# kakao/buffalo

Measured on NVIDIA H100. Metric: interactions/sec (nnz/s) ALS d=128, higher is better.
Workload: dtype f32

## Files before the change

### buffalo_b200/csrc/als_fast.cuh

```cuda
#pragma once
#include <algorithm>
#include <map>

#include "als_explicit.cuh"
#include "als_generic.cuh"
#include "als_tc.cuh"
#include "bfl_common.cuh"

namespace bfl {

constexpr int FAST_WARPS = 16;
constexpr int FAST_THREADS = FAST_WARPS * 32;
constexpr int FAST_NCLASS = 8;
constexpr int FAST_NR_CAP = 12288;

struct FastClass { int W, K, res, cap; };
__host__ __device__ inline FastClass fast_class(int c) {
    switch (c) {
        case 0: return {1, 1, 1, 32};
        case 1: return {1, 2, 1, 64};
        case 2: return {2, 2, 1, 128};
        case 3: return {4, 2, 1, 256};
        case 4: return {8, 2, 1, 512};
        case 5: return {16, 3, 1, 1536};
        case 6: return {16, 1, 0, FAST_NR_CAP};
        default: return {0, 0, 0, 0x7fffffff};
    }
}
__host__ __device__ inline int fast_class_of(int64_t n) {
    if (n <= 32) return 0;
    if (n <= 64) return 1;
    if (n <= 128) return 2;
    if (n <= 256) return 3;
    if (n <= 512) return 4;
    if (n <= 1536) return 5;
    if (n <= FAST_NR_CAP) return 6;
    return 7;
}

__host__ __device__ inline int fast_route(int64_t n, int long_regather) {
    const int c = fast_class_of(n);
    return (long_regather && c == 5) ? 6 : c;
}

__global__ void fast_count_kernel(const int64_t* __restrict__ indptr, int64_t row_begin, int64_t row_end,
                                  unsigned int* __restrict__ counts, int long_regather) {
    __shared__ unsigned int c[FAST_NCLASS];
    if (threadIdx.x < FAST_NCLASS) c[threadIdx.x] = 0;
    __syncthreads();
    for (int64_t r = row_begin + (int64_t)blockIdx.x * blockDim.x + threadIdx.x; r < row_end;
         r += (int64_t)gridDim.x * blockDim.x) {
        const int64_t n = indptr[r] - (r == 0 ? 0 : indptr[r - 1]);
        if (n > 0) atomicAdd(&c[fast_route(n, long_regather)], 1u);
    }
    __syncthreads();
    if (threadIdx.x < FAST_NCLASS && c[threadIdx.x]) atomicAdd(counts + threadIdx.x, c[threadIdx.x]);
}

__global__ void fast_fill_kernel(const int64_t* __restrict__ indptr, int64_t row_begin, int64_t row_end,
                                 unsigned int* __restrict__ cursors, int32_t* __restrict__ lists, int long_regather) {
    for (int64_t r = row_begin + (int64_t)blockIdx.x * blockDim.x + threadIdx.x; r < row_end;
         r += (int64_t)gridDim.x * blockDim.x) {
        const int64_t n = indptr[r] - (r == 0 ? 0 : indptr[r - 1]);
        if (n > 0) {
            const unsigned int pos = atomicAdd(cursors + fast_route(n, long_regather), 1u);
            lists[pos] = (int32_t)r;
        }
    }
}

template <int W>
__device__ __forceinline__ void team_sync(int team) {
    if (W == 1) {
        __syncwarp();
    } else {
        asm volatile("bar.sync %0, %1;" ::"r"(team + 1), "r"(32 * W) : "memory");
    }
}

__device__ __forceinline__ float4 ldg4(const float* p) { return __ldg(reinterpret_cast<const float4*>(p)); }
__device__ __forceinline__ float4 lds4(const float* p) { return *reinterpret_cast<const float4*>(p); }

__device__ __forceinline__ float2 ffma2(float2 a, float2 b, float2 c) {
    return make_float2(fmaf(a.x, b.x, c.x), fmaf(a.y, b.y, c.y));
}
__device__ __forceinline__ float2 fmul2(float2 a, float2 b) { return make_float2(__fmul_rn(a.x, b.x), __fmul_rn(a.y, b.y)); }

struct V8 { float2 v[4]; };

__device__ __forceinline__ V8 v8_zero() {
    V8 r;
#pragma unroll
    for (int k = 0; k < 4; ++k) r.v[k] = make_float2(0.f, 0.f);
    return r;
}
__device__ __forceinline__ V8 v8_from(float4 lo, float4 hi) {
    V8 r;
    r.v[0] = make_float2(lo.x, lo.y); r.v[1] = make_float2(lo.z, lo.w);
    r.v[2] = make_float2(hi.x, hi.y); r.v[3] = make_float2(hi.z, hi.w);
    return r;
}
__device__ __forceinline__ V8 v8_lds(const float* p) { return v8_from(lds4(p), lds4(p + 4)); }
__device__ __forceinline__ V8 v8_ldg(const float* p) { return v8_from(ldg4(p), ldg4(p + 4)); }
__device__ __forceinline__ float v8_dot(const V8& q, const V8& x) {
    float2 s = fmul2(q.v[0], x.v[0]);
#pragma unroll
    for (int k = 1; k < 4; ++k) s = ffma2(q.v[k], x.v[k], s);
    return s.x + s.y;
}
__device__ __forceinline__ void v8_axpy(V8& acc, float cf, const V8& q) {
    const float2 c2 = make_float2(cf, cf);
#pragma unroll
    for (int k = 0; k < 4; ++k) acc.v[k] = ffma2(c2, q.v[k], acc.v[k]);
}

__device__ __forceinline__ float transposed_reduce8(const V8& acc, int la) {
    const bool h4 = la & 4, h2 = la & 2, h1 = la & 1;
    const float2 s0 = h4 ? acc.v[0] : acc.v[2], s1 = h4 ? acc.v[1] : acc.v[3];
    const float2 k0 = h4 ? acc.v[2] : acc.v[0], k1 = h4 ? acc.v[3] : acc.v[1];
    float2 v0, v1;
    v0.x = k0.x + __shfl_xor_sync(FULL, s0.x, 16);
    v0.y = k0.y + __shfl_xor_sync(FULL, s0.y, 16);
    v1.x = k1.x + __shfl_xor_sync(FULL, s1.x, 16);
    v1.y = k1.y + __shfl_xor_sync(FULL, s1.y, 16);
    const float2 s = h2 ? v0 : v1, k = h2 ? v1 : v0;
    float2 u;
    u.x = k.x + __shfl_xor_sync(FULL, s.x, 8);
    u.y = k.y + __shfl_xor_sync(FULL, s.y, 8);
    return (h1 ? u.y : u.x) + __shfl_xor_sync(FULL, h1 ? u.x : u.y, 4);
}

__device__ __forceinline__ float sum_over_b(float s) {
    s += __shfl_xor_sync(FULL, s, 1);
    s += __shfl_xor_sync(FULL, s, 2);
    return s;
}

__device__ __forceinline__ void cp_async16(void* smem_dst, const void* gsrc) {
    asm volatile("cp.async.cg.shared.global [%0], [%1], 16;" ::"r"(smem_u32(smem_dst)), "l"(gsrc) : "memory");
}
__device__ __forceinline__ void cp_async_commit() { asm volatile("cp.async.commit_group;" ::: "memory"); }
__device__ __forceinline__ void cp_async_wait_all() { asm volatile("cp.async.wait_group 0;" ::: "memory"); }
__device__ __forceinline__ void prefetch_l2(const void* p) { asm volatile("prefetch.global.L2 [%0];" ::"l"(p)); }

__host__ __device__ inline size_t fast_team_floats(int D, int W, int cap) { return (size_t)D + 96 * W + 96 + 3 * (size_t)cap; }
__host__ __device__ inline size_t fast_smem_bytes(int D, int W, int K, int KS, bool res, bool gsm, int cap) {
    return sizeof(float) * ((gsm ? (size_t)D * (D + 4) : 0) + (res ? (size_t)FAST_WARPS * (K + KS) * 8 * 128 : 0) +
                            (FAST_WARPS / W) * fast_team_floats(D, W, cap));
}

template <int W, int K, int KS, bool RES, bool GSM, bool DET = false>
__global__ void __launch_bounds__(FAST_THREADS, 1) als_ialspp_team_kernel(AlsArgs a, int cap) {
    extern __shared__ __align__(16) float smem[];
    constexpr int TEAMS = FAST_WARPS / W;
    constexpr int KT = K + KS;
    const int D = a.D, ld = a.ld, GP = GSM ? D + 4 : D, NB = D >> 5;
    const int tid = threadIdx.x, lane = tid & 31;
    const int warp = __shfl_sync(FULL, tid >> 5, 0);
// ... 411 lines not shown
        const int g7 = (int)std::min<int64_t>((n7 + 127) / 128, 1024);
        if (BFL_OK != fb->chunk_end.reserve((size_t)n7)) return BFL_ERR_CUDA;
        tc::tc_chunk_counts_kernel<<<g7, 128, 0, st>>>(a0.indptr, list7, n7, TC_SPLIT, fb->chunk_end.p);
        BFL_LAUNCHED();
        int rc = inclusive_scan_i64(fb->chunk_end.p, fb->chunk_end.p, n7, st);
        if (rc != BFL_OK) return rc;
        fb->h_chunk_end.resize((size_t)n7);
        BFL_CUDA(cudaMemcpyAsync(fb->h_chunk_end.data(), fb->chunk_end.p, sizeof(long long) * (size_t)n7, cudaMemcpyDeviceToHost, st));
        BFL_CUDA(cudaStreamSynchronize(st));
        const long long total = fb->h_chunk_end.back();
        if (BFL_OK != fb->items.reserve(3 * (size_t)total)) return BFL_ERR_CUDA;
        tc::tc_fill_items_scanned_kernel<<<g7, 128, 0, st>>>(list7, n7, fb->chunk_end.p, fb->items.p);
        BFL_LAUNCHED();
        fb->n_items = (int64_t)total;
        fb->items_split_class = split_min_class;
        fb->items_det = true;
        fb->det_batches.clear();
    }
    const size_t sf = tc::scratch_floats<D>(), sfb = sf * sizeof(float);
    if (!cache.det_budget) {
        size_t free_b = 0, total_b = 0;
        BFL_CUDA(cudaMemGetInfo(&free_b, &total_b));
        cache.det_budget = std::max<size_t>(std::min<size_t>(free_b / 4, (size_t)2 << 30), 2 * sfb);
    }
    const long long* ce = fb->h_chunk_end.data();
    if (fb->det_batches.empty() || fb->det_batches_budget != cache.det_budget) {
        fb->det_batches.assign(1, 0);
        size_t used = 0;
        for (int64_t i = 0; i < n7; ++i) {
            const size_t cost = (size_t)(ce[i] - (i ? ce[i - 1] : 0) + 1) * sfb;
            if (used && used + cost > cache.det_budget) {
                fb->det_batches.push_back(i);
                used = 0;
            }
            used += cost;
        }
        fb->det_batches.push_back(n7);
        fb->det_batches_budget = cache.det_budget;
    }
    int64_t max_rows = 0, max_chunks = 0;
    for (size_t b = 0; b + 1 < fb->det_batches.size(); ++b) {
        const int64_t i = fb->det_batches[b], j = fb->det_batches[b + 1];
        max_rows = std::max(max_rows, j - i);
        max_chunks = std::max<int64_t>(max_chunks, ce[j - 1] - (i ? ce[i - 1] : 0));
    }
    if (BFL_OK != cache.scratch.reserve(sf * (size_t)max_rows) || BFL_OK != cache.chunk_scratch.reserve(sf * (size_t)max_chunks))
        BFL_FAIL(BFL_ERR_CUDA, "deterministic ALS: cannot allocate the split-row scratch (" +
                                   std::to_string((sfb * (size_t)(max_rows + max_chunks)) >> 20) +
                                   " MB); lower _b200_det_scratch_mb or free device memory");
    const int nf4 = (int)((a0.compute_loss && a0.axis == 1 ? sf : (size_t)D * D + D) / 4);
    for (size_t b = 0; b + 1 < fb->det_batches.size(); ++b) {
        const int64_t i = fb->det_batches[b], j = fb->det_batches[b + 1];
        const int64_t chunk0 = i ? ce[i - 1] : 0, nchunks = ce[j - 1] - chunk0;
        int rc = tc::tc_launch_partial<D>(a0, fb->items.p + 3 * chunk0, nchunks, cache.chunk_scratch.p, nchunks, TC_SPLIT,
                                          num_sms, st, true);
        if (rc != BFL_OK) return rc;
        for (int64_t r = i; r < j; r += 65535) {
            const dim3 grid((nf4 + 255) / 256, (unsigned)std::min<int64_t>(65535, j - r));
            tc::tc_chunk_reduce_kernel<<<grid, 256, 0, st>>>(cache.chunk_scratch.p, fb->chunk_end.p, r, chunk0, sf, nf4,
                                                             cache.scratch.p + (size_t)(r - i) * sf);
            BFL_LAUNCHED();
        }
        rc = launch_explicit_solve(a0, list7 + i, j - i, cache.scratch.p, det_loss, num_sms, st);
        if (rc != BFL_OK) return rc;
    }
    return BFL_OK;
}

inline int fast_als_launch(const AlsArgs& a0, FastCache& cache, int num_sms, cudaStream_t st,
                           const int32_t** leftover_rows, int64_t* leftover_count, int tc_min_class, int split_min_class,
                           int long_regather = 0, bool det = false) {
    const bool det_loss = det && a0.loss && a0.compute_loss;
    *leftover_rows = nullptr;
    *leftover_count = 0;
    const int64_t nrows = a0.row_end - a0.row_begin;
    FastBinKey key{a0.indptr, a0.row_begin, a0.row_end};
    FastBins* fb = nullptr;
    auto it = cache.bins.find(key);
    if (it == cache.bins.end()) {
        if (cache.bins.size() >= 256) cache.clear();
        fb = new FastBins();
        if (BFL_OK != fb->lists.reserve((size_t)nrows) || BFL_OK != fb->counters.reserve(2 * FAST_NCLASS)) {
            delete fb;
            return BFL_ERR_CUDA;
        }
        BFL_CUDA(cudaMemsetAsync(fb->counters.p, 0, 2 * FAST_NCLASS * sizeof(unsigned int), st));
        const int grid = (int)std::min<int64_t>((nrows + 255) / 256, (int64_t)num_sms * 8);
        fast_count_kernel<<<grid, 256, 0, st>>>(a0.indptr, a0.row_begin, a0.row_end, fb->counters.p, long_regather);
        BFL_LAUNCHED();
        BFL_CUDA(cudaMemcpyAsync(fb->count, fb->counters.p, FAST_NCLASS * sizeof(unsigned int), cudaMemcpyDeviceToHost, st));
        BFL_CUDA(cudaStreamSynchronize(st));
        fb->offset[0] = 0;
        for (int c = 0; c < FAST_NCLASS; ++c) fb->offset[c + 1] = fb->offset[c] + fb->count[c];
        BFL_CUDA(cudaMemcpyAsync(fb->counters.p + FAST_NCLASS, fb->offset, FAST_NCLASS * sizeof(unsigned int),
                                 cudaMemcpyHostToDevice, st));
        fast_fill_kernel<<<grid, 256, 0, st>>>(a0.indptr, a0.row_begin, a0.row_end, fb->counters.p + FAST_NCLASS,
                                               fb->lists.p, long_regather);
        BFL_LAUNCHED();
        cache.bins[key] = fb;
    } else {
        fb = it->second;
    }
    tc_min_class = std::min(tc_min_class, split_min_class);
    const bool has_split = split_min_class < FAST_NCLASS && fb->offset[FAST_NCLASS] > fb->offset[split_min_class];
    if (has_split && det) {
        const int64_t n7 = fb->offset[FAST_NCLASS] - fb->offset[split_min_class];
        const int32_t* list7 = fb->lists.p + fb->offset[split_min_class];
        const int rc = a0.D == 128
                           ? fast_split_rows_det<128>(a0, cache, fb, list7, n7, split_min_class, det_loss, num_sms, st)
                           : fast_split_rows_det<256>(a0, cache, fb, list7, n7, split_min_class, det_loss, num_sms, st);
        if (rc != BFL_OK) return rc;
    }
    if (has_split && !det) {
        const int64_t n7 = fb->offset[FAST_NCLASS] - fb->offset[split_min_class];
        const int32_t* list7 = fb->lists.p + fb->offset[split_min_class];
        if (fb->n_items < 0 || fb->items_split_class != split_min_class) {
            if (BFL_OK != fb->item_counter.reserve(2)) return BFL_ERR_CUDA;
            BFL_CUDA(cudaMemsetAsync(fb->item_counter.p, 0, 2 * sizeof(unsigned long long), st));
            const int g7 = (int)std::min<int64_t>((n7 + 127) / 128, 1024);
            tc::tc_count_items_kernel<<<g7, 128, 0, st>>>(a0.indptr, list7, n7, TC_SPLIT, fb->item_counter.p);
            BFL_LAUNCHED();
            unsigned long long total = 0;
            BFL_CUDA(cudaMemcpyAsync(&total, fb->item_counter.p, sizeof(total), cudaMemcpyDeviceToHost, st));
            BFL_CUDA(cudaStreamSynchronize(st));
            if (BFL_OK != fb->items.reserve(3 * (size_t)total)) return BFL_ERR_CUDA;
            tc::tc_fill_items_kernel<<<g7, 128, 0, st>>>(a0.indptr, list7, n7, TC_SPLIT, fb->item_counter.p + 1, fb->items.p);
            BFL_LAUNCHED();
            fb->n_items = (int64_t)total;
            fb->items_split_class = split_min_class;
        }
        const size_t sf = a0.D == 128 ? tc::scratch_floats<128>() : tc::scratch_floats<256>();
        if (BFL_OK != cache.scratch.reserve(sf * (size_t)n7)) return BFL_ERR_CUDA;
        int rc = a0.D == 128
                     ? tc::tc_launch_partial<128>(a0, fb->items.p, fb->n_items, cache.scratch.p, n7, TC_SPLIT, num_sms, st)
                     : tc::tc_launch_partial<256>(a0, fb->items.p, fb->n_items, cache.scratch.p, n7, TC_SPLIT, num_sms, st);
        if (rc != BFL_OK) return rc;
        rc = launch_explicit_solve(a0, list7, n7, cache.scratch.p, false, num_sms, st);
        if (rc != BFL_OK) return rc;
    }
    if (tc_min_class < split_min_class && fb->offset[split_min_class] > fb->offset[tc_min_class]) {
        AlsArgs a = a0;
        a.row_list = fb->lists.p;
        a.row_begin = fb->offset[tc_min_class];
        a.row_end = fb->offset[split_min_class];
        const int rc = tc::tc_launch(a, num_sms, st, det_loss);
        if (rc != BFL_OK) return rc;
    }
    for (int c = 0; c < std::min(FAST_NCLASS - 1, tc_min_class); ++c) {
        if (!fb->count[c]) continue;
        AlsArgs a = a0;
        a.row_list = fb->lists.p;
        a.row_begin = fb->offset[c];
        a.row_end = fb->offset[c + 1];
        const FastClass fc = fast_class(c);
        int rc = BFL_OK;
        const bool gsm = a.D <= 128;
        switch (c) {
            case 0: rc = gsm ? fast_launch_class<1, 1, 0, true, true>(a, fc.cap, num_sms, st, det_loss)
                             : fast_launch_class<1, 1, 0, true, false>(a, fc.cap, num_sms, st, det_loss); break;
            case 1: rc = gsm ? fast_launch_class<1, 2, 0, true, true>(a, fc.cap, num_sms, st, det_loss)
                             : fast_launch_class<1, 2, 0, true, false>(a, fc.cap, num_sms, st, det_loss); break;
            case 2: rc = gsm ? fast_launch_class<2, 2, 0, true, true>(a, fc.cap, num_sms, st, det_loss)
                             : fast_launch_class<2, 2, 0, true, false>(a, fc.cap, num_sms, st, det_loss); break;
            case 3: rc = gsm ? fast_launch_class<4, 2, 0, true, true>(a, fc.cap, num_sms, st, det_loss)
                             : fast_launch_class<4, 2, 0, true, false>(a, fc.cap, num_sms, st, det_loss); break;
            case 4: rc = gsm ? fast_launch_class<8, 2, 0, true, true>(a, fc.cap, num_sms, st, det_loss)
                             : fast_launch_class<8, 2, 0, true, false>(a, fc.cap, num_sms, st, det_loss); break;
            case 5: rc = fast_launch_class<16, 2, 1, true, false>(a, fc.cap, num_sms, st, det_loss); break;
            case 6: rc = gsm ? fast_launch_class<16, 1, 0, false, true>(a, fc.cap, num_sms, st, det_loss)
                             : fast_launch_class<16, 1, 0, false, false>(a, fc.cap, num_sms, st, det_loss); break;
        }
        if (rc != BFL_OK) return rc;
    }
    if (split_min_class >= FAST_NCLASS && fb->count[FAST_NCLASS - 1]) {
        *leftover_rows = fb->lists.p + fb->offset[FAST_NCLASS - 1];
        *leftover_count = fb->count[FAST_NCLASS - 1];
    }
    return BFL_OK;
}

}
```

### buffalo_b200/csrc/als_tc.cuh

```cuda
#pragma once
#include "als_generic.cuh"
#include "bfl_common.cuh"
#include <type_traits>

#include "sm90_ptx.cuh"

namespace bfl {
namespace tc {

using namespace sm90;

constexpr int N_CONV = 4, KH = N_CONV / 4;
constexpr int W_EPI = 0, W_MMA = 4, W_CONV = 8, W_PLAN = W_CONV + N_CONV;
constexpr int WARPS = 16, THREADS = WARPS * 32;
constexpr int REG_MMA = 200, REG_PLAN = 4 * 128 - 128 - 128 - REG_MMA;
constexpr int NXS = 8;
constexpr int PT = 2;
constexpr int NR = 2;
constexpr int NO = 2;
constexpr int GATHER_AHEAD = 1;
constexpr int NPG = 8, NP = NPG * PT;
constexpr int NBV = 8;
template <int D>
struct Cfg {
    static constexpr int TILE = D == 128 ? 32 : 16;
    static constexpr int NF = D / 128;
    static constexpr int LBO = D * 16;
    static constexpr int OP_BYTES = TILE * D * 2;
};
constexpr uint32_t F_FIRST = 1u << 8, F_LAST = 1u << 9, F_NEG = 1u << 10, F_STOP = 1u << 11;

__device__ __forceinline__ int msw(int c) { return ((c >> 1) & 3) << 3; }

template <int D>
struct Smem {
    static constexpr int TILE = Cfg<D>::TILE;
    alignas(1024) unsigned char op[NO][PT][2][Cfg<D>::OP_BYTES];
    alignas(128) float raw[NR][PT][TILE * D];
    alignas(128) float mat[128 * 128];
    alignas(16) float bvec[NBV][KH][D];
    alignas(16) float sumq[NBV][KH][D];
    alignas(16) float xs[NXS][D];
    alignas(16) float pv[4][32];
    alignas(16) float dl[4][32];
    alignas(16) float sws[NP][TILE];
    alignas(16) float wv[NP][TILE];
    alignas(16) int32_t keys[NP][TILE];
    float wsum[NBV][KH];
    uint32_t meta_raw[NP];
    uint32_t meta_op[NO][PT];
    int badrow[NXS];
    alignas(8) uint64_t plan_full[NPG], plan_empty[NPG], raw_full[NR], raw_empty[NR], op_full[NO], op_empty[NO];
    alignas(8) uint64_t acc_full, acc_empty, x_full[NXS], d_full[4];
};
template <int D>
struct SmemDet : Smem<D> {
    double lossp[NXS][4][2];
};

struct TcArgs {
    AlsArgs a;
    const int32_t* items;
    float* scratch;
    int64_t split;
    int pass;
    int debug;
};

template <int D>
__host__ __device__ constexpr size_t scratch_floats() { return (size_t)D * D + 2 * D + 4; }

__global__ void tc_absmax_kernel(const float* __restrict__ p, size_t n, unsigned int* __restrict__ out) {
    float m = 0.f;
    const size_t gtid = (size_t)blockIdx.x * blockDim.x + threadIdx.x, gsz = (size_t)gridDim.x * blockDim.x;
    const size_t lead = min(n, (size_t)(((16 - ((uintptr_t)p & 15)) & 15) / 4));
    const size_t n4 = (n - lead) / 4;
    const float4* p4 = reinterpret_cast<const float4*>(p + lead);
    for (size_t i = gtid; i < n4; i += gsz) {
        const float4 v = __ldg(p4 + i);
        m = fmaxf(fmaxf(m, fmaxf(fabsf(v.x), fabsf(v.y))), fmaxf(fabsf(v.z), fabsf(v.w)));
    }
    for (size_t i = gtid; i < lead; i += gsz) m = fmaxf(m, fabsf(p[i]));
    for (size_t i = lead + n4 * 4 + gtid; i < n; i += gsz) m = fmaxf(m, fabsf(p[i]));
    for (int o = 16; o > 0; o >>= 1) m = fmaxf(m, __shfl_xor_sync(FULL, m, o));
    if ((threadIdx.x & 31) == 0 && m > 0.f) atomicMax(out, __float_as_uint(m));
}
__global__ void tc_scale_kernel(const unsigned int* __restrict__ ymax, const unsigned int* __restrict__ vmax, float alpha,
                                float* __restrict__ out) {
    const float y = __uint_as_float(*ymax), w = __uint_as_float(*vmax) * fabsf(alpha);
    const float top = y * sqrtf(w);
    int e = 0;
    if (top > 0.f && isfinite(top)) {
        int ex;
        frexpf(top, &ex);
        e = 15 - ex;
    }
    e = max(-60, min(60, e));
    out[0] = ldexpf(1.f, e);
    out[1] = ldexpf(1.f, -2 * e);
}

template <int D, bool PARTIAL, bool LOSS1, bool DET = false>
__global__ void __launch_bounds__(THREADS, 1) als_tc_kernel(TcArgs ta) {
    static_assert(D == 128 || (D == 256 && PARTIAL), "fused row solve: d = 128; split-row mode: d = 128 or 256");
    constexpr int TILE = Cfg<D>::TILE, NF = Cfg<D>::NF, LBO = Cfg<D>::LBO;
    extern __shared__ __align__(1024) unsigned char smem_raw_[];
    Smem<D>& S = *reinterpret_cast<Smem<D>*>(smem_raw_);
    [[maybe_unused]] SmemDet<D>& SD = *reinterpret_cast<SmemDet<D>*>(smem_raw_);
    const AlsArgs& a = ta.a;
    const int tid = threadIdx.x, lane = tid & 31;
    const int warp = __shfl_sync(FULL, tid >> 5, 0);

    if (tid == 0) {
        for (int i = 0; i < NR; ++i) {
            mbar_init(&S.raw_full[i], N_CONV);
            mbar_init(&S.raw_empty[i], N_CONV);
        }
        for (int i = 0; i < NPG; ++i) {
            mbar_init(&S.plan_full[i], 1);
            mbar_init(&S.plan_empty[i], N_CONV);
        }
        for (int i = 0; i < NO; ++i) {
            mbar_init(&S.op_full[i], N_CONV);
            mbar_init(&S.op_empty[i], 4);
        }
        mbar_init(&S.acc_full, 4);
        mbar_init(&S.acc_empty, 4);
        for (int b = 0; b < 4; ++b) mbar_init(&S.d_full[b], 1);
        for (int i = 0; i < NXS; ++i) {
            mbar_init(&S.x_full[i], 4);
            S.badrow[i] = 0;
        }
        mbar_init_fence();
    }
    __syncthreads();
    const float scale = __ldg(a.tc_scales), inv2 = __ldg(a.tc_scales + 1);

    const int64_t nitems = a.row_end - a.row_begin;
    const int64_t my_first = (int64_t)blockIdx.x;
    const int64_t stride = gridDim.x;

    auto item_info = [&](int64_t it, int& row, int64_t& beg, int64_t& n, int& slot) {
        if (PARTIAL) {
            const int32_t* p = ta.items + 3 * (a.row_begin + it);
            row = p[0];
            const int64_t rb = row == 0 ? 0 : a.indptr[row - 1];
            const int64_t rn = a.indptr[row] - rb;
            beg = rb + (int64_t)p[1] * ta.split;
            n = min(ta.split, rn - (int64_t)p[1] * ta.split);
            slot = DET ? (int)it : p[2];
        } else {
            row = a.row_list[a.row_begin + it];
            beg = row == 0 ? 0 : a.indptr[row - 1];
            n = a.indptr[row] - beg;
            slot = 0;
        }
    };

    if (warp >= W_PLAN) {
        setmaxnreg_dec<REG_PLAN>();
        if (warp != W_PLAN) return;
        uint32_t gsl = 0, rph = 0, pe = 0;
        auto tile_begin = [&]() -> uint32_t {
            if (pe == 0) mbar_wait_idle(&S.plan_empty[gsl], rph ^ 1u);
            return gsl * PT + pe;
        };
        auto tile_end = [&]() {
            if (++pe == PT) {
                if (lane == 0) mbar_arrive(&S.plan_full[gsl]);
                pe = 0;
                if (++gsl == NPG) { gsl = 0; rph ^= 1u; }
            }
        };
        auto emit = [&](unsigned mask, uint32_t flags, int32_t key, float w) {
            const int cnt = __popc(mask);
            const int slot = __popc(mask & ((1u << lane) - 1u));
            const uint32_t rs = tile_begin();
            if ((mask >> lane) & 1u) {
                S.keys[rs][slot] = key;
                S.sws[rs][slot] = sqrtf(fabsf(w)) * scale;
                S.wv[rs][slot] = w;
            } else {
                const int zslot = cnt + lane - slot;
                if (zslot < TILE) {
                    S.sws[rs][zslot] = 0.f;
                    S.wv[rs][zslot] = 0.f;
                }
            }
            if (lane == 0) S.meta_raw[rs] = (uint32_t)cnt | flags;
            __syncwarp();
            tile_end();
        };
        constexpr int SC = 4, SCN = SC * TILE;
        const bool inl = lane < TILE;
        auto load_id = [&](int64_t it, int& row, int& chunk) {
            row = -1;
            chunk = 0;
            if (it < nitems) {
                if (PARTIAL) {
                    const int32_t* p = ta.items + 3 * (a.row_begin + it);
                    row = p[0];
                    chunk = p[1];
                } else {
                    row = a.row_list[a.row_begin + it];
                }
            }
        };
        auto load_span = [&](int row, int chunk, const int32_t*& kp, const float*& vp, int& n) {
            kp = a.keys;
            vp = a.vals;
            n = 0;
            if (row >= 0) {
                const int64_t rb = row == 0 ? 0 : a.indptr[row - 1];
                const int64_t rn = a.indptr[row] - rb;
                int64_t beg = rb;
                n = (int)rn;
                if (PARTIAL) {
                    beg = rb + (int64_t)chunk * ta.split;
                    n = (int)min(ta.split, rn - (int64_t)chunk * ta.split);
                }
                kp = a.keys + (beg - a.shift);
                vp = a.vals + (beg - a.shift);
            }
        };
        auto load_sc = [&](const int32_t* kp, const float* vp, int n, int c0, int32_t (&key)[SC], float (&w)[SC]) {
#pragma unroll
            for (int s = 0; s < SC; ++s) {
                const int idx = c0 + s * TILE + lane;
                const bool ok = inl && idx < n;
                key[s] = ok ? kp[idx] : 0;
                w[s] = ok ? vp[idx] * a.alpha : 0.f;
            }
        };
        auto emit_sc = [&](int n, int c0, const int32_t (&key)[SC], const float (&w)[SC]) {
            bool neg = false;
#pragma unroll
            for (int s = 0; s < SC; ++s) neg |= w[s] < 0.f;
            if (!__any_sync(FULL, neg)) {
#pragma unroll
                for (int s = 0; s < SC; ++s) {
                    const int t0 = c0 + s * TILE;
                    if (t0 < n) {
                        const uint32_t meta = (uint32_t)min(TILE, n - t0) | (t0 == 0 ? F_FIRST : 0u) | (t0 + TILE >= n ? F_LAST : 0u);
                        const uint32_t rs = tile_begin();
                        if (inl) {
                            float sq;
                            asm("sqrt.approx.ftz.f32 %0, %1;" : "=f"(sq) : "f"(w[s]));
                            S.keys[rs][lane] = key[s];
                            S.sws[rs][lane] = sq * scale;
                            S.wv[rs][lane] = w[s];
                        }
                        if (lane == 0) S.meta_raw[rs] = meta;
                        __syncwarp();
                        tile_end();
// ... 434 lines not shown
            if (++os == NO) { os = 0; oph ^= 1u; }
        }
    } else {
        const int q = warp & 3;
        const int j = q * 32 + lane;
        float* pv = S.pv[q];
        double l_nume = 0.0, l_deno = 0.0;
        const float tol = a.tol;
        if constexpr (PARTIAL) {
            int row = 0, slot = 0, nrow = 0, nslot = 0;
            int64_t beg, n = 0, nbeg, nn = 0;
            if (my_first < nitems) item_info(my_first, row, beg, n, slot);
            for (int64_t seq = 0; my_first + seq * stride < nitems; ++seq) {
                const int64_t nit = my_first + (seq + 1) * stride;
                if (nit < nitems) item_info(nit, nrow, nbeg, nn, nslot);
                const uint32_t aph = (uint32_t)(seq & 1);
                const uint32_t bs = (uint32_t)(seq & (NBV - 1));
                mbar_wait_idle(&S.acc_full, aph);
                float* sc = ta.scratch + (size_t)slot * scratch_floats<D>();
                if constexpr (DET) {
                    if (ta.pass == 0) {
                        for (int jj = j; jj < D; jj += 128) {
                            sc[(size_t)D * D + jj] = S.bvec[bs][0][jj] + (KH == 2 ? S.bvec[bs][KH - 1][jj] : 0.f);
                            if (LOSS1) sc[(size_t)D * D + D + jj] = S.sumq[bs][0][jj] + (KH == 2 ? S.sumq[bs][KH - 1][jj] : 0.f);
                        }
                        if (LOSS1 && j < 4)
                            sc[(size_t)D * D + 2 * D + j] = j == 0 ? S.wsum[bs][0] + (KH == 2 ? S.wsum[bs][KH - 1] : 0.f) : 0.f;
                    }
                } else if (ta.pass == 0) {
                    for (int jj = j; jj < D; jj += 128) {
                        atomicAdd(sc + (size_t)D * D + jj, S.bvec[bs][0][jj] + (KH == 2 ? S.bvec[bs][KH - 1][jj] : 0.f));
                        if (LOSS1) atomicAdd(sc + (size_t)D * D + D + jj, S.sumq[bs][0][jj] + (KH == 2 ? S.sumq[bs][KH - 1][jj] : 0.f));
                    }
                    if (LOSS1 && j == 0) atomicAdd(sc + (size_t)D * D + 2 * D, S.wsum[bs][0] + (KH == 2 ? S.wsum[bs][KH - 1] : 0.f));
                }
                __syncwarp();
                if (lane == 0) mbar_arrive(&S.acc_empty);
                row = nrow; slot = nslot; n = nn;
            }
        } else {
            auto row_of = [&](int64_t sq) -> int {
                const int64_t it = my_first + sq * stride;
                return it < nitems ? a.row_list[a.row_begin + it] : -1;
            };
            auto len_of = [&](int row) -> float {
                if (row < 0 || !a.compute_loss) return 0.f;
                return (float)(a.indptr[row] - (row == 0 ? 0 : a.indptr[row - 1]));
            };
            int row = (ta.debug & 16) ? -1 : row_of(0), row1 = row_of(1), row2 = row_of(2);
            float xj = row >= 0 ? a.X[(int64_t)row * a.ld + j] : 0.f;
            float x1 = row1 >= 0 ? a.X[(int64_t)row1 * a.ld + j] : 0.f;
            float nlen = len_of(row), nlen1 = len_of(row1);
            if (row >= 0) {
                S.xs[0][j] = xj;
                __syncwarp();
                if (lane == 0) mbar_arrive(&S.x_full[0]);
            }
            auto mat = [&](int c) -> float { return S.mat[c * 128 + (j ^ msw(c))]; };
            for (int64_t seq = 0; row >= 0; ++seq) {
                const int row3 = row_of(seq + 3);
                const float x2 = row2 >= 0 ? a.X[(int64_t)row2 * a.ld + j] : 0.f;
                const float nlen2 = len_of(row2);
                if (row1 >= 0) {
                    S.xs[(seq + 1) & (NXS - 1)][j] = x1;
                    __syncwarp();
                    if (lane == 0) mbar_arrive(&S.x_full[(seq + 1) & (NXS - 1)]);
                }
                const uint32_t aph = (uint32_t)(seq & 1);
                const uint32_t bs = (uint32_t)(seq & (NBV - 1));
                const uint32_t xsl = (uint32_t)(seq & (NXS - 1));
                const float* xs = S.xs[xsl];
                mbar_wait(&S.x_full[xsl], (uint32_t)((seq / NXS) & 1));
                mbar_wait_idle(&S.acc_full, aph);
                if (ta.debug & 8) {
                    __syncwarp();
                    if (lane == 0) mbar_arrive(&S.acc_empty);
                    row = row1; row1 = row2; row2 = row3;
                    xj = x1; x1 = x2;
                    continue;
                }
                const float bj = S.bvec[bs][0][j] + (KH == 2 ? S.bvec[bs][KH - 1][j] : 0.f);
                double ln_row = 0.0, ld_row = 0.0;
                float hM = 0.f;
                float md[32];
#pragma unroll
                for (int c = 0; c < D / 32; ++c) {
                    float h0 = 0.f, h1 = 0.f;
#pragma unroll
                    for (int i = 0; i < 32; i += 4) {
                        const float4 x4 = *reinterpret_cast<const float4*>(xs + c * 32 + i);
                        const float m0 = mat(c * 32 + i), m1 = mat(c * 32 + i + 1), m2 = mat(c * 32 + i + 2), m3 = mat(c * 32 + i + 3);
                        h0 = fmaf(m0, x4.x, h0); h1 = fmaf(m1, x4.y, h1);
                        h0 = fmaf(m2, x4.z, h0); h1 = fmaf(m3, x4.w, h1);
                        if (c == q) { md[i] = m0; md[i + 1] = m1; md[i + 2] = m2; md[i + 3] = m3; }
                    }
                    hM += h0 + h1;
                }
                if (a.compute_loss) {
                    const float kappa = a.adaptive_reg ? nlen : 1.0f;
                    double t = (double)(kappa * a.reg * xj * xj);
                    if (a.axis == 1) {
                        t += (double)xj * (double)hM - (double)(a.reg * xj * xj) -
                             2.0 * (double)xj * ((double)bj + (double)S.sumq[bs][0][j] + (KH == 2 ? (double)S.sumq[bs][KH - 1][j] : 0.0));
                        if (j == 0) {
                            const double ws = (double)S.wsum[bs][0] + (KH == 2 ? (double)S.wsum[bs][KH - 1] : 0.0);
                            t += (double)nlen + ws;
                            l_deno += (double)a.Y_rows + ws;
                        }
                    }
                    if constexpr (DET) {
                        ln_row = warp_sum_d(t);
                        ld_row = l_deno;
                        l_deno = 0.0;
                        if (q < 3 && lane == 0) {
                            SD.lossp[xsl][q][0] = ln_row;
                            SD.lossp[xsl][q][1] = ld_row;
                        }
                    } else {
                        l_nume += t;
                    }
                }
                float h = hM - bj;
#pragma unroll 1
                for (int B = 0; B < q; ++B) {
                    float mv[32];
#pragma unroll
                    for (int i = 0; i < 32; ++i) mv[i] = mat(B * 32 + i);
                    mbar_wait(&S.d_full[B], aph);
                    float u0 = 0.f, u1 = 0.f;
#pragma unroll
                    for (int i = 0; i < 32; i += 4) {
                        const float4 d4 = *reinterpret_cast<const float4*>(&S.dl[B][i]);
                        u0 = fmaf(mv[i], d4.x, u0);
                        u1 = fmaf(mv[i + 1], d4.y, u1);
                        u0 = fmaf(mv[i + 2], d4.z, u0);
                        u1 = fmaf(mv[i + 3], d4.w, u1);
                    }
                    h -= u0 + u1;
                }
                if constexpr (DET) {
                    if (q == 3 && lane == 0 && a.loss && a.compute_loss) {
                        double sn = SD.lossp[xsl][0][0], sd = SD.lossp[xsl][0][1];
#pragma unroll
                        for (int w = 1; w < 3; ++w) {
                            sn += SD.lossp[xsl][w][0];
                            sd += SD.lossp[xsl][w][1];
                        }
                        a.loss[2 * (int64_t)row] = sn + ln_row;
                        a.loss[2 * (int64_t)row + 1] = sd + ld_row;
                    }
                }
                __syncwarp();
                if (lane == 0) mbar_arrive(&S.acc_empty);
                float xv = 0.f;
                {
                    float r = h, p = h;
                    float rsold = warp_sum(r * r);
                    bool act = rsold > tol;
#pragma unroll 1
                    for (int step = 0; step < 3; ++step) {
                        pv[lane] = p;
                        __syncwarp();
                        float a0 = 0.f, a1 = 0.f, a2 = 0.f, a3 = 0.f;
#pragma unroll
                        for (int i = 0; i < 32; i += 4) {
                            const float4 p4 = *reinterpret_cast<const float4*>(pv + i);
                            a0 = fmaf(md[i], p4.x, a0); a1 = fmaf(md[i + 1], p4.y, a1);
                            a2 = fmaf(md[i + 2], p4.z, a2); a3 = fmaf(md[i + 3], p4.w, a3);
                        }
                        __syncwarp();
                        const float Ap = (a0 + a1) + (a2 + a3);
                        const float pAp = warp_sum(p * Ap);
                        const float ss = act ? __fdividef(rsold, pAp) : 0.f;
                        xv = fmaf(ss, p, xv);
                        r = fmaf(-ss, Ap, r);
                        const float rsnew = warp_sum(r * r);
                        act = act && !(rsnew < tol);
                        if (act) p = fmaf(__fdividef(rsnew, rsold), p, r);
                        rsold = act ? rsnew : rsold;
                    }
                }
                float v = xj - xv;
                const bool badw = __any_sync(FULL, !isfinite(v));
                a.X[(int64_t)row * a.ld + j] = v;
                for (int pr = 0; pr < a.n_peer; ++pr) a.peerX[pr][(int64_t)row * a.ld + j] = v;
                if (q < 3) {
                    S.dl[q][lane] = xv;
                    if (badw && lane == 0) atomicOr(&S.badrow[xsl], 1);
                    __syncwarp();
                    if (lane == 0) mbar_arrive(&S.d_full[q]);
                }
                if (q == 3) {
                    const bool bad = badw || (S.badrow[xsl] != 0);
                    if (bad) {
#pragma unroll
                        for (int c = 0; c < 4; ++c) {
                            a.X[(int64_t)row * a.ld + c * 32 + lane] = 0.f;
                            for (int pr = 0; pr < a.n_peer; ++pr) a.peerX[pr][(int64_t)row * a.ld + c * 32 + lane] = 0.f;
                        }
                        __syncwarp();
                        if (lane == 0) S.badrow[xsl] = 0;
                    }
                }
                row = row1; row1 = row2; row2 = row3;
                xj = x1; x1 = x2;
                nlen = nlen1; nlen1 = nlen2;
            }
            if (!DET && a.loss && a.compute_loss) {
                l_nume = warp_sum_d(l_nume);
                l_deno = warp_sum_d(l_deno);
                if (lane == 0 && (l_nume != 0.0 || l_deno != 0.0)) {
                    atomicAdd(a.loss, l_nume);
                    atomicAdd(a.loss + 1, l_deno);
                }
            }
        }
    }
}

inline bool tc_applicable(int optimizer_code, int d, int vdim, int block_size) {
    return optimizer_code == 8 && d == 128 && vdim == 128 && block_size == 32;
}
inline bool tc_split_applicable(int optimizer_code, int d, int vdim, int block_size) {
    return optimizer_code == 8 && (d == 128 || d == 256) && vdim == d && block_size == 32;
}

inline int tc_note_absmax(const float* p, size_t n, unsigned int* out, int num_sms, cudaStream_t st) {
    BFL_CUDA(cudaMemsetAsync(out, 0, sizeof(unsigned int), st));
    if (n == 0) return BFL_OK;
    const int grid = (int)std::min<size_t>((n / 4 + 255) / 256 + 1, (size_t)num_sms * 8);
    tc_absmax_kernel<<<grid, 256, 0, st>>>(p, n, out);
    BFL_LAUNCHED();
    return BFL_OK;
}
inline int tc_update_scale(const unsigned int* ymax, const unsigned int* vmax, float alpha, float* scales, cudaStream_t st) {
    tc_scale_kernel<<<1, 1, 0, st>>>(ymax, vmax, alpha, scales);
    BFL_LAUNCHED();
    return BFL_OK;
}

__global__ void tc_count_items_kernel(const int64_t* __restrict__ indptr, const int32_t* __restrict__ list, int64_t nrows,
                                      int64_t split, unsigned long long* total) {
    for (int64_t i = (int64_t)blockIdx.x * blockDim.x + threadIdx.x; i < nrows; i += (int64_t)gridDim.x * blockDim.x) {
        const int row = list[i];
        const int64_t n = indptr[row] - (row == 0 ? 0 : indptr[row - 1]);
        atomicAdd(total, (unsigned long long)((n + split - 1) / split));
    }
}
__global__ void tc_fill_items_kernel(const int64_t* __restrict__ indptr, const int32_t* __restrict__ list, int64_t nrows,
                                     int64_t split, unsigned long long* cursor, int32_t* __restrict__ items) {
    for (int64_t i = (int64_t)blockIdx.x * blockDim.x + threadIdx.x; i < nrows; i += (int64_t)gridDim.x * blockDim.x) {
        const int row = list[i];
        const int64_t n = indptr[row] - (row == 0 ? 0 : indptr[row - 1]);
        const int64_t nc = (n + split - 1) / split;
        const unsigned long long pos = atomicAdd(cursor, (unsigned long long)nc);
        for (int64_t c = 0; c < nc; ++c) {
            items[3 * (pos + c) + 0] = row;
            items[3 * (pos + c) + 1] = (int32_t)c;
            items[3 * (pos + c) + 2] = (int32_t)i;
        }
    }
}

__global__ void tc_chunk_counts_kernel(const int64_t* __restrict__ indptr, const int32_t* __restrict__ list, int64_t nrows,
                                       int64_t split, long long* __restrict__ counts) {
    for (int64_t i = (int64_t)blockIdx.x * blockDim.x + threadIdx.x; i < nrows; i += (int64_t)gridDim.x * blockDim.x) {
        const int row = list[i];
        const int64_t n = indptr[row] - (row == 0 ? 0 : indptr[row - 1]);
        counts[i] = (n + split - 1) / split;
    }
}
__global__ void tc_fill_items_scanned_kernel(const int32_t* __restrict__ list, int64_t nrows,
                                             const long long* __restrict__ chunk_end, int32_t* __restrict__ items) {
    for (int64_t i = (int64_t)blockIdx.x * blockDim.x + threadIdx.x; i < nrows; i += (int64_t)gridDim.x * blockDim.x) {
        const int64_t pos = i == 0 ? 0 : chunk_end[i - 1], nc = chunk_end[i] - pos;
        for (int64_t c = 0; c < nc; ++c) {
            items[3 * (pos + c) + 0] = list[i];
            items[3 * (pos + c) + 1] = (int32_t)c;
            items[3 * (pos + c) + 2] = (int32_t)i;
        }
    }
}

__global__ void __launch_bounds__(256) tc_chunk_reduce_kernel(const float* __restrict__ chunks, const long long* __restrict__ chunk_end,
                                                              int64_t row0, int64_t chunk0, size_t slot_floats, int nf4,
                                                              float* __restrict__ rows_out) {
    const int64_t i = row0 + blockIdx.y;
    const int64_t c0 = (i == 0 ? 0 : chunk_end[i - 1]) - chunk0, c1 = chunk_end[i] - chunk0;
    float4* out = reinterpret_cast<float4*>(rows_out + (size_t)blockIdx.y * slot_floats);
    for (int e = blockIdx.x * blockDim.x + threadIdx.x; e < nf4; e += gridDim.x * blockDim.x) {
        float4 acc = __ldg(reinterpret_cast<const float4*>(chunks + (size_t)c0 * slot_floats) + e);
        for (int64_t c = c0 + 1; c < c1; ++c) {
            const float4 v = __ldg(reinterpret_cast<const float4*>(chunks + (size_t)c * slot_floats) + e);
            acc.x = __fadd_rn(acc.x, v.x);
            acc.y = __fadd_rn(acc.y, v.y);
            acc.z = __fadd_rn(acc.z, v.z);
            acc.w = __fadd_rn(acc.w, v.w);
        }
        out[e] = acc;
    }
}

template <int D>
int tc_launch_partial(const AlsArgs& a, const int32_t* items, int64_t nitems, float* scratch, int64_t nslots,
                      int64_t split, int num_sms, cudaStream_t st, bool det = false) {
    if (nitems <= 0) return BFL_OK;
    if (!a.tc_scales) BFL_FAIL(BFL_ERR_STATE, "tensor-core ALS kernel: operand scale not prepared");
    TcArgs ta;
    ta.a = a;
    ta.a.row_begin = 0;
    ta.a.row_end = nitems;
    ta.items = items;
    ta.scratch = scratch;
    ta.split = split;
    ta.debug = 0;
    if (!det) BFL_CUDA(cudaMemsetAsync(scratch, 0, sizeof(float) * scratch_floats<D>() * (size_t)nslots, st));
    const size_t smem = sizeof(Smem<D>);
    const int grid = (int)std::min<int64_t>(nitems, (int64_t)num_sms);
    for (ta.pass = 0; ta.pass < (D == 128 ? 1 : 3); ++ta.pass) {
        if (det && a.compute_loss && a.axis == 1) {
            BFL_CUDA(cudaFuncSetAttribute(als_tc_kernel<D, true, true, true>, cudaFuncAttributeMaxDynamicSharedMemorySize, (int)smem));
            als_tc_kernel<D, true, true, true><<<grid, THREADS, smem, st>>>(ta);
        } else if (det) {
            BFL_CUDA(cudaFuncSetAttribute(als_tc_kernel<D, true, false, true>, cudaFuncAttributeMaxDynamicSharedMemorySize, (int)smem));
            als_tc_kernel<D, true, false, true><<<grid, THREADS, smem, st>>>(ta);
        } else if (a.compute_loss && a.axis == 1) {
            BFL_CUDA(cudaFuncSetAttribute(als_tc_kernel<D, true, true>, cudaFuncAttributeMaxDynamicSharedMemorySize, (int)smem));
            als_tc_kernel<D, true, true><<<grid, THREADS, smem, st>>>(ta);
        } else {
            BFL_CUDA(cudaFuncSetAttribute(als_tc_kernel<D, true, false>, cudaFuncAttributeMaxDynamicSharedMemorySize, (int)smem));
            als_tc_kernel<D, true, false><<<grid, THREADS, smem, st>>>(ta);
        }
        BFL_LAUNCHED();
    }
// ... 39 lines not shown
```

Baseline: 1.433 billion.

## Add warp-per-row tensor-core kernel for short rows (33-64 nnz)

Adds a dedicated kernel for the 33-64-nonzero row class at d=128. Each warp solves one row using mma.sync with fp16 hi/lo split operands to build 32x32 diagonal Gram blocks. It runs a block-wise conjugate-gradient update, staging Y slices through cp.async. The aim is to replace the generic FMA-based fast-class kernel for these rows with tensor-core accumulation, at the cost of split-precision error and heavy shared memory per warp. The existing CG inner loop is moved into a shared helper.

```diff
diff --git a/buffalo_b200/csrc/als_fast.cuh b/buffalo_b200/csrc/als_fast.cuh
--- a/buffalo_b200/csrc/als_fast.cuh
+++ b/buffalo_b200/csrc/als_fast.cuh
@@ -4,6 +4,7 @@
 
 #include "als_explicit.cuh"
 #include "als_generic.cuh"
+#include "als_short.cuh"
 #include "als_tc.cuh"
 #include "bfl_common.cuh"
 
@@ -721,6 +722,11 @@
         a.row_list = fb->lists.p;
         a.row_begin = fb->offset[c];
         a.row_end = fb->offset[c + 1];
+        if (c == 1 && a.D == 128 && a.tc_scales) {
+            const int rc = tcs::short_launch(a, num_sms, st, det_loss);
+            if (rc != BFL_OK) return rc;
+            continue;
+        }
         const FastClass fc = fast_class(c);
         int rc = BFL_OK;
         const bool gsm = a.D <= 128;
diff --git a/buffalo_b200/csrc/als_short.cuh b/buffalo_b200/csrc/als_short.cuh
--- /dev/null
+++ b/buffalo_b200/csrc/als_short.cuh
@@ -0,0 +1,373 @@
+#pragma once
+#include <cuda_fp16.h>
+
+#include "als_generic.cuh"
+#include "als_tc.cuh"
+#include "bfl_common.cuh"
+#include "sm90_ptx.cuh"
+
+namespace bfl {
+namespace tcs {
+
+using namespace sm90;
+
+constexpr int SD = 128;
+constexpr int SPITCH = 36;
+
+template <int NMAX>
+struct ShortCfg {
+    static constexpr int WARPS = NMAX == 32 ? 16 : 10;
+};
+
+template <int NMAX>
+struct ShortWarp {
+    alignas(16) float stg[NMAX][SPITCH];
+    alignas(16) float ms[32][33];
+    alignas(16) float xs[SD];
+    alignas(16) float yui[NMAX];
+    alignas(16) float wv[NMAX];
+    alignas(16) float sws[NMAX];
+    alignas(16) int32_t ks[NMAX];
+    alignas(16) float hv[32];
+    alignas(16) float dl[32];
+    alignas(16) float pv[32];
+};
+template <int NMAX>
+struct ShortSmem {
+    uint4 gf[8][8][2][32];
+    ShortWarp<NMAX> w[ShortCfg<NMAX>::WARPS];
+    unsigned int gmax;
+};
+
+__device__ __forceinline__ void mma_f16(float (&c)[4], uint4 a, uint32_t b0, uint32_t b1) {
+    asm volatile("mma.sync.aligned.m16n8k16.row.col.f32.f16.f16.f32 {%0,%1,%2,%3}, {%4,%5,%6,%7}, {%8,%9}, {%0,%1,%2,%3};"
+                 : "+f"(c[0]), "+f"(c[1]), "+f"(c[2]), "+f"(c[3])
+                 : "r"(a.x), "r"(a.y), "r"(a.z), "r"(a.w), "r"(b0), "r"(b1));
+}
+__device__ __forceinline__ void mma_split(float (&c)[4], uint4 ah, uint4 al, uint32_t bh0, uint32_t bh1, uint32_t bl0,
+                                          uint32_t bl1) {
+    mma_f16(c, ah, bh0, bh1);
+    mma_f16(c, ah, bl0, bl1);
+    mma_f16(c, al, bh0, bh1);
+}
+__device__ __forceinline__ int pow2_exp(float top) {
+    int e = 0;
+    if (top > 0.f && isfinite(top)) {
+        int ex;
+        frexpf(top, &ex);
+        e = max(-100, min(100, 15 - ex));
+    }
+    return e;
+}
+__device__ __forceinline__ float warp_max(float v) {
+#pragma unroll
+    for (int o = 16; o > 0; o >>= 1) v = fmaxf(v, __shfl_xor_sync(FULL, v, o));
+    return v;
+}
+
+template <int NMAX, bool DET = false>
+__global__ void __launch_bounds__(ShortCfg<NMAX>::WARPS * 32, 1) als_short_tc_kernel(AlsArgs a) {
+    constexpr int WARPS = ShortCfg<NMAX>::WARPS;
+    extern __shared__ __align__(16) unsigned char smem_raw_[];
+    ShortSmem<NMAX>& S = *reinterpret_cast<ShortSmem<NMAX>*>(smem_raw_);
+    const int tid = threadIdx.x, lane = tid & 31;
+    const int warp = __shfl_sync(FULL, tid >> 5, 0);
+    const int g = lane >> 2, t = lane & 3;
+    ShortWarp<NMAX>& W = S.w[warp];
+    const int ld = a.ld;
+    const float reg = a.reg, tol = a.tol;
+    const float sc = __ldg(a.tc_scales), inv2 = __ldg(a.tc_scales + 1), s2 = sc * sc;
+
+    if (tid == 0) S.gmax = 0u;
+    __syncthreads();
+    {
+        float m = 0.f;
+        for (int e = tid; e < SD * SD; e += WARPS * 32) {
+            const int r = e >> 7, c = e & (SD - 1);
+            m = fmaxf(m, fabsf(__ldg(a.G + e) + (r == c ? reg : 0.f)));
+        }
+        m = warp_max(m);
+        if (lane == 0 && m > 0.f) atomicMax(&S.gmax, __float_as_uint(m));
+    }
+    __syncthreads();
+    const int eg = pow2_exp(__uint_as_float(S.gmax));
+    const float gsc = ldexpf(1.f, eg);
+    for (int f = tid; f < 8 * 8 * 32; f += WARPS * 32) {
+        const int i = f >> 8, s = (f >> 5) & 7, l = f & 31;
+        const int r0 = 16 * i + (l >> 2), c0 = 16 * s + 2 * (l & 3);
+        auto ge = [&](int r, int c) { return (__ldg(a.G + r * SD + c) + (r == c ? reg : 0.f)) * gsc; };
+        uint4 h, lo;
+        split_f16x2(make_float2(ge(r0, c0), ge(r0, c0 + 1)), h.x, lo.x);
+        split_f16x2(make_float2(ge(r0 + 8, c0), ge(r0 + 8, c0 + 1)), h.y, lo.y);
+        split_f16x2(make_float2(ge(r0, c0 + 8), ge(r0, c0 + 9)), h.z, lo.z);
+        split_f16x2(make_float2(ge(r0 + 8, c0 + 8), ge(r0 + 8, c0 + 9)), h.w, lo.w);
+        S.gf[i][s][0][l] = h;
+        S.gf[i][s][1][l] = lo;
+    }
+    __syncthreads();
+
+    auto dense = [&](int Bq) {
+        __syncwarp();
+        const float4 x4 = *reinterpret_cast<const float4*>(W.xs + 4 * lane);
+        const int ex = pow2_exp(warp_max(fmaxf(fmaxf(fabsf(x4.x), fabsf(x4.y)), fmaxf(fabsf(x4.z), fabsf(x4.w)))));
+        const float xsc = ldexpf(1.f, ex);
+        float c[4][4];
+#pragma unroll
+        for (int i = 0; i < 4; ++i)
+#pragma unroll
+            for (int e = 0; e < 4; ++e) c[i][e] = 0.f;
+#pragma unroll
+        for (int s = 0; s < 8; ++s) {
+            const float2 x0 = *reinterpret_cast<const float2*>(W.xs + 16 * s + 2 * t);
+            const float2 x8 = *reinterpret_cast<const float2*>(W.xs + 16 * s + 2 * t + 8);
+            uint32_t bh0, bl0, bh1, bl1;
+            split_f16x2(f2mul(x0, make_float2(xsc, xsc)), bh0, bl0);
+            split_f16x2(f2mul(x8, make_float2(xsc, xsc)), bh1, bl1);
+#pragma unroll
+            for (int i = 0; i < 2; ++i)
+                mma_split(c[i + 2 * (s & 1)], S.gf[2 * Bq + i][s][0][lane], S.gf[2 * Bq + i][s][1][lane], bh0, bh1, bl0, bl1);
+        }
+#pragma unroll
+        for (int e = 0; e < 4; ++e) {
+            c[0][e] += c[2][e];
+            c[1][e] += c[3][e];
+        }
+        const float u = ldexpf(1.f, -(eg + ex));
+        if (t == 0) {
+            W.hv[g] = c[0][0] * u;
+            W.hv[g + 8] = c[0][2] * u;
+            W.hv[g + 16] = c[1][0] * u;
+            W.hv[g + 24] = c[1][2] * u;
+        }
+        __syncwarp();
+    };
+
+    double l_nume = 0.0, l_deno = 0.0;
+    const int64_t stride = (int64_t)gridDim.x * WARPS;
+    for (int64_t ri = a.row_begin + (int64_t)blockIdx.x * WARPS + warp; ri < a.row_end; ri += stride) {
+        const int row = __shfl_sync(FULL, a.row_list[ri], 0);
+        const int64_t beg = row == 0 ? 0 : a.indptr[row - 1];
+        const int n = __shfl_sync(FULL, (int)(a.indptr[row] - beg), 0);
+        const int npad = (n + 15) & ~15, nks = npad >> 4;
+        float* xrow = a.X + (int64_t)row * ld;
+        __syncwarp();
+        {
+            const int32_t k0 = a.keys[beg - a.shift];
+#pragma unroll
+            for (int c = lane; c < NMAX; c += 32) {
+                const bool ok = c < n;
+                const float w = ok ? a.vals[beg - a.shift + c] * a.alpha : 0.f;
+                W.ks[c] = ok ? a.keys[beg - a.shift + c] : k0;
+                W.wv[c] = w;
+                W.sws[c] = sqrtf(fabsf(w)) * sc;
+                W.yui[c] = 0.f;
+            }
+        }
+        const float4 x4 = *reinterpret_cast<const float4*>(xrow + 4 * lane);
+        *reinterpret_cast<float4*>(W.xs + 4 * lane) = x4;
+        __syncwarp();
+        auto stage = [&](int B) {
+            for (int c = lane; c < npad * 8; c += 32) {
+                const int k = c >> 3, ch = c & 7;
+                cp_async16_cg(&W.stg[k][ch * 4], a.Y + (int64_t)W.ks[k] * ld + B * 32 + ch * 4);
+            }
+            cp_async_commit();
+        };
+        stage(0);
+
+        {
+            float4 xr[8];
+#pragma unroll
+            for (int c = 0; c < 8; ++c) xr[c] = *reinterpret_cast<const float4*>(W.xs + 16 * c + 4 * t);
+#pragma unroll 2
+            for (int i = 0; 8 * i < n; ++i) {
+                const int k = g + 8 * i;
+                const float* yp = a.Y + (int64_t)W.ks[k] * ld + 4 * t;
+                float dot = 0.f;
+#pragma unroll
+                for (int c = 0; c < 8; ++c) {
+                    const float4 q = __ldg(reinterpret_cast<const float4*>(yp + 16 * c));
+                    dot = fmaf(q.x, xr[c].x, dot);
+                    dot = fmaf(q.y, xr[c].y, dot);
+                    dot = fmaf(q.z, xr[c].z, dot);
+                    dot = fmaf(q.w, xr[c].w, dot);
+                }
+                dot += __shfl_xor_sync(FULL, dot, 1);
+                dot += __shfl_xor_sync(FULL, dot, 2);
+                if (t == 0 && k < n) {
+                    W.yui[k] = dot;
+                    if (a.compute_loss && a.axis == 1) {
+                        const float av = W.wv[k];
+                        l_nume += -(double)(dot * dot) + (double)((dot - 1.f) * (dot - 1.f)) * (1.0 + (double)av);
+                        l_deno += (double)av;
+                    }
+                }
+            }
+        }
+        if (a.compute_loss) {
+            const float xx = warp_sum(x4.x * x4.x + x4.y * x4.y + x4.z * x4.z + x4.w * x4.w);
+            float xgx = 0.f;
+            if (a.axis == 1) {
+#pragma unroll 1
+                for (int Bq = 0; Bq < SD / 32; ++Bq) {
+                    dense(Bq);
+                    xgx = fmaf(W.xs[32 * Bq + lane], W.hv[lane], xgx);
+                }
+                xgx = warp_sum(xgx) - reg * xx;
+            }
+            if (lane == 0) {
+                l_nume += (double)((a.adaptive_reg ? (float)n : 1.0f) * reg * xx);
+                if (a.axis == 1) {
+                    l_nume += (double)xgx;
+                    l_deno += (double)a.Y_rows;
+                }
+            }
+            if (DET && a.loss) {
+                l_nume = warp_sum_d(l_nume);
+                l_deno = warp_sum_d(l_deno);
+                if (lane == 0) {
+                    a.loss[2 * (int64_t)row] = l_nume;
+                    a.loss[2 * (int64_t)row + 1] = l_deno;
+                }
+            }
+            if (DET) l_nume = l_deno = 0.0;
+        }
+        __syncwarp();
+
+#pragma unroll 1
+        for (int B = 0; B < SD / 32; ++B) {
+            dense(B);
+            cp_async_wait_group<0>();
+            __syncwarp();
+            float acc[2][4][4];
+            {
+                const float u = ldexpf(1.f, -eg) * s2;
+#pragma unroll
+                for (int i = 0; i < 2; ++i)
+#pragma unroll
+                    for (int j = 0; j < 4; ++j) {
+                        if (i == 0 && j >= 2) continue;
+                        const uint4 h4 = S.gf[2 * B + i][2 * B + (j >> 1)][0][lane], l4 = S.gf[2 * B + i][2 * B + (j >> 1)][1][lane];
+                        const uint32_t hr[2] = {(j & 1) ? h4.z : h4.x, (j & 1) ? h4.w : h4.y};
+                        const uint32_t lr[2] = {(j & 1) ? l4.z : l4.x, (j & 1) ? l4.w : l4.y};
+#pragma unroll
+                        for (int h = 0; h < 2; ++h) {
+                            const float2 hf = __half22float2(*reinterpret_cast<const __half2*>(&hr[h]));
+                            const float2 lf = __half22float2(*reinterpret_cast<const __half2*>(&lr[h]));
+                            acc[i][j][2 * h] = (hf.x + lf.x) * u;
+                            acc[i][j][2 * h + 1] = (hf.y + lf.y) * u;
+                        }
+                    }
+            }
+#pragma unroll 1
+            for (int s = 0; s < nks; ++s) {
+                const int k0 = 16 * s + 2 * t;
+                const float4 sw = make_float4(W.sws[k0], W.sws[k0 + 1], W.sws[k0 + 8], W.sws[k0 + 9]);
+                const uint32_t sg0 = (W.wv[k0] < 0.f ? 0x8000u : 0u) | (W.wv[k0 + 1] < 0.f ? 0x80000000u : 0u);
+                const uint32_t sg8 = (W.wv[k0 + 8] < 0.f ? 0x8000u : 0u) | (W.wv[k0 + 9] < 0.f ? 0x80000000u : 0u);
+                uint32_t bh[4][2], bl[4][2];
+#pragma unroll
+                for (int j = 0; j < 4; ++j) {
+                    const int f = 8 * j + g;
+                    split_f16x2(make_float2(W.stg[k0][f] * sw.x, W.stg[k0 + 1][f] * sw.y), bh[j][0], bl[j][0]);
+                    split_f16x2(make_float2(W.stg[k0 + 8][f] * sw.z, W.stg[k0 + 9][f] * sw.w), bh[j][1], bl[j][1]);
+                }
+#pragma unroll
+                for (int i = 0; i < 2; ++i) {
+                    const uint4 ah = make_uint4(bh[2 * i][0] ^ sg0, bh[2 * i + 1][0] ^ sg0, bh[2 * i][1] ^ sg8, bh[2 * i + 1][1] ^ sg8);
+                    const uint4 al = make_uint4(bl[2 * i][0] ^ sg0, bl[2 * i + 1][0] ^ sg0, bl[2 * i][1] ^ sg8, bl[2 * i + 1][1] ^ sg8);
+#pragma unroll
+                    for (int j = 0; j < 4; ++j) {
+                        if (i == 0 && j >= 2) continue;
+                        mma_split(acc[i][j], ah, al, bh[j][0], bh[j][1], bl[j][0], bl[j][1]);
+                    }
+                }
+            }
+#pragma unroll
+            for (int i = 0; i < 2; ++i)
+#pragma unroll
+                for (int j = 0; j < 4; ++j) {
+                    if (i == 0 && j >= 2) continue;
+#pragma unroll
+                    for (int e = 0; e < 4; ++e) {
+                        const int r = 16 * i + g + 8 * (e >> 1), c = 8 * j + 2 * t + (e & 1);
+                        const float v = acc[i][j][e] * inv2;
+                        W.ms[r][c] = v;
+                        if (i == 1 && j < 2) W.ms[c][r] = v;
+                    }
+                }
+            __syncwarp();
+            float sp0 = 0.f, sp1 = 0.f, sp2 = 0.f, sp3 = 0.f;
+#pragma unroll 4
+            for (int k = 0; k < npad; k += 4) {
+                const float4 y4 = *reinterpret_cast<const float4*>(W.yui + k);
+                const float4 w4 = *reinterpret_cast<const float4*>(W.wv + k);
+                sp0 = fmaf((y4.x - 1.0f) * w4.x, W.stg[k][lane], sp0);
+                sp1 = fmaf((y4.y - 1.0f) * w4.y, W.stg[k + 1][lane], sp1);
+                sp2 = fmaf((y4.z - 1.0f) * w4.z, W.stg[k + 2][lane], sp2);
+                sp3 = fmaf((y4.w - 1.0f) * w4.w, W.stg[k + 3][lane], sp3);
+            }
+            const float sp = (sp0 + sp1) + (sp2 + sp3);
+            float md[32];
+#pragma unroll
+            for (int i = 0; i < 32; ++i) md[i] = W.ms[lane][i];
+            const float xv = tc::block_cg3(md, W.hv[lane] + sp, W.pv, tol);
+            W.xs[32 * B + lane] -= xv;
+            W.dl[lane] = xv;
+            __syncwarp();
+            if (B + 1 < SD / 32) {
+#pragma unroll
+                for (int k = lane; k < NMAX; k += 32) {
+                    if (k < npad) {
+                        float u0 = 0.f, u1 = 0.f;
+#pragma unroll
+                        for (int c = 0; c < 32; c += 4) {
+                            const float4 q4 = *reinterpret_cast<const float4*>(&W.stg[k][c]);
+                            const float4 d4 = *reinterpret_cast<const float4*>(W.dl + c);
+                            u0 = fmaf(q4.x, d4.x, u0);
+                            u1 = fmaf(q4.y, d4.y, u1);
+                            u0 = fmaf(q4.z, d4.z, u0);
+                            u1 = fmaf(q4.w, d4.w, u1);
+                        }
+                        W.yui[k] -= u0 + u1;
+                    }
+                }
+                __syncwarp();
+                stage(B + 1);
+            }
+        }
+        float4 xo = *reinterpret_cast<const float4*>(W.xs + 4 * lane);
+        const bool bad = __any_sync(FULL, !(isfinite(xo.x) && isfinite(xo.y) && isfinite(xo.z) && isfinite(xo.w)));
+        if (bad) xo = make_float4(0.f, 0.f, 0.f, 0.f);
+        *reinterpret_cast<float4*>(xrow + 4 * lane) = xo;
+        for (int pr = 0; pr < a.n_peer; ++pr) *reinterpret_cast<float4*>(a.peerX[pr] + (int64_t)row * ld + 4 * lane) = xo;
+    }
+    if (!DET && a.loss && a.compute_loss) {
+        l_nume = warp_sum_d(l_nume);
+        l_deno = warp_sum_d(l_deno);
+        if (lane == 0 && (l_nume != 0.0 || l_deno != 0.0)) {
+            atomicAdd(a.loss, l_nume);
+            atomicAdd(a.loss + 1, l_deno);
+        }
+    }
+}
+
+template <int NMAX, bool DET>
+int short_launch_n(const AlsArgs& a, int num_sms, cudaStream_t st) {
+    constexpr int WARPS = ShortCfg<NMAX>::WARPS;
+    const size_t smem = sizeof(ShortSmem<NMAX>);
+    BFL_CUDA(cudaFuncSetAttribute(als_short_tc_kernel<NMAX, DET>, cudaFuncAttributeMaxDynamicSharedMemorySize, (int)smem));
+    const int64_t nrows = a.row_end - a.row_begin;
+    const int grid = (int)std::min<int64_t>((nrows + WARPS - 1) / WARPS, (int64_t)num_sms);
+    als_short_tc_kernel<NMAX, DET><<<grid, WARPS * 32, smem, st>>>(a);
+    BFL_LAUNCHED();
+    return BFL_OK;
+}
+inline int short_launch(const AlsArgs& a, int num_sms, cudaStream_t st, bool det_loss) {
+    if (a.row_end <= a.row_begin) return BFL_OK;
+    if (!a.tc_scales) BFL_FAIL(BFL_ERR_STATE, "short-row tensor-core ALS kernel: operand scale not prepared");
+    return det_loss ? short_launch_n<64, true>(a, num_sms, st) : short_launch_n<64, false>(a, num_sms, st);
+}
+
+}
+}
diff --git a/buffalo_b200/csrc/als_tc.cuh b/buffalo_b200/csrc/als_tc.cuh
--- a/buffalo_b200/csrc/als_tc.cuh
+++ b/buffalo_b200/csrc/als_tc.cuh
@@ -100,6 +100,37 @@
     out[1] = ldexpf(1.f, -2 * e);
 }
 
+__device__ __forceinline__ float block_cg3(const float (&md)[32], float h, float* pv, float tol) {
+    const int lane = threadIdx.x & 31;
+    float xv = 0.f;
+    float r = h, p = h;
+    float rsold = warp_sum(r * r);
+    bool act = rsold > tol;
+#pragma unroll 1
+    for (int step = 0; step < 3; ++step) {
+        pv[lane] = p;
+        __syncwarp();
+        float a0 = 0.f, a1 = 0.f, a2 = 0.f, a3 = 0.f;
+#pragma unroll
+        for (int i = 0; i < 32; i += 4) {
+            const float4 p4 = *reinterpret_cast<const float4*>(pv + i);
+            a0 = fmaf(md[i], p4.x, a0); a1 = fmaf(md[i + 1], p4.y, a1);
+            a2 = fmaf(md[i + 2], p4.z, a2); a3 = fmaf(md[i + 3], p4.w, a3);
+        }
+        __syncwarp();
+        const float Ap = (a0 + a1) + (a2 + a3);
+        const float pAp = warp_sum(p * Ap);
+        const float ss = act ? __fdividef(rsold, pAp) : 0.f;
+        xv = fmaf(ss, p, xv);
+        r = fmaf(-ss, Ap, r);
+        const float rsnew = warp_sum(r * r);
+        act = act && !(rsnew < tol);
+        if (act) p = fmaf(__fdividef(rsnew, rsold), p, r);
+        rsold = act ? rsnew : rsold;
+    }
+    return xv;
+}
+
 template <int D, bool PARTIAL, bool LOSS1, bool DET = false>
 __global__ void __launch_bounds__(THREADS, 1) als_tc_kernel(TcArgs ta) {
     static_assert(D == 128 || (D == 256 && PARTIAL), "fused row solve: d = 128; split-row mode: d = 128 or 256");
@@ -840,34 +871,7 @@
                 }
                 __syncwarp();
                 if (lane == 0) mbar_arrive(&S.acc_empty);
-                float xv = 0.f;
-                {
-                    float r = h, p = h;
-                    float rsold = warp_sum(r * r);
-                    bool act = rsold > tol;
-#pragma unroll 1
-                    for (int step = 0; step < 3; ++step) {
-                        pv[lane] = p;
-                        __syncwarp();
-                        float a0 = 0.f, a1 = 0.f, a2 = 0.f, a3 = 0.f;
-#pragma unroll
-                        for (int i = 0; i < 32; i += 4) {
-                            const float4 p4 = *reinterpret_cast<const float4*>(pv + i);
-                            a0 = fmaf(md[i], p4.x, a0); a1 = fmaf(md[i + 1], p4.y, a1);
-                            a2 = fmaf(md[i + 2], p4.z, a2); a3 = fmaf(md[i + 3], p4.w, a3);
-                        }
-                        __syncwarp();
-                        const float Ap = (a0 + a1) + (a2 + a3);
-                        const float pAp = warp_sum(p * Ap);
-                        const float ss = act ? __fdividef(rsold, pAp) : 0.f;
-                        xv = fmaf(ss, p, xv);
-                        r = fmaf(-ss, Ap, r);
-                        const float rsnew = warp_sum(r * r);
-                        act = act && !(rsnew < tol);
-                        if (act) p = fmaf(__fdividef(rsnew, rsold), p, r);
-                        rsold = act ? rsnew : rsold;
-                    }
-                }
+                const float xv = block_cg3(md, h, pv, tol);
                 float v = xj - xv;
                 const bool badw = __any_sync(FULL, !isfinite(v));
                 a.X[(int64_t)row * a.ld + j] = v;
```

Result: faster. 1.454 billion (median of 6 runs) (+1.5%).
